# hulu/statsd-router

Hardware: AMD Instinct MI355X
Metric: M metrics/s parsed+hashed, device-resident (GiB/s and HBM roofline alongside) (higher is better)
Workload: dtype u64

## Files before the change

### statsd-router_amd/csrc/route_kernel.hpp

```cpp
#pragma once

#include <hip/hip_runtime.h>
#include <stdint.h>

#include "../../include/sr_route.h"

namespace srk {

constexpr int kBlock = 256;
constexpr int kLaneBytes = 64;
constexpr int kTile = kBlock * kLaneBytes;
constexpr int kOverlay = 16;
constexpr int kNone = 0x1FFFF;
constexpr int kSpinBudget = 1 << 14;
constexpr uint32_t kFlagAgg = 1u, kFlagIncl = 2u;
constexpr uint16_t kRoutePending = 0xFFFCu;
constexpr uint32_t kRouteDefer = 0xFFFBu;
constexpr uint64_t K = 65599ull;
constexpr int kPowLo = 64, kPowHi = 24;
constexpr int kPowInv = 4;

enum : unsigned {
    KV_UNIFORM = 0,
    KV_SEGMENTS = 1u << 22,
    KV_CHUNKS = 1u << 23,
    KV_ALIVE = 1u << 28,
    KV_PICKS = 1u << 29,
    KV_DEFER1 = 1u << 31,
    KV_DEAD1 = 1u << 27,
    KV_HIST1 = 1u << 20,
};
enum : unsigned {
    ABL_NONE = 0,
    ABL_NO_LOOKBACK = 1u << 0,
    ABL_NO_LINES = 1u << 1,
    ABL_NO_PROLOGUE = 1u << 2,
    ABL_LOAD_ONLY = 1u << 4,
    ABL_STAMPS = 1u << 5,
    ABL_NO_HASH = 1u << 8,
    ABL_FAKE_BASE = 1u << 12,
    ABL_NO_MID_BASE = 1u << 21,
};
enum : unsigned { CH_ABL_NO_U = 1u << 24, CH_ABL_NO_SUF = 1u << 25, CH_ABL_NO_EMIT = 1u << 26 };

constexpr unsigned kKvBits = KV_SEGMENTS | KV_CHUNKS | KV_ALIVE | KV_PICKS | KV_DEFER1 | KV_DEAD1 | KV_HIST1;
constexpr unsigned kAblBits = ABL_NO_LOOKBACK | ABL_NO_LINES | ABL_NO_PROLOGUE | ABL_LOAD_ONLY | ABL_STAMPS |
                              ABL_NO_HASH | ABL_FAKE_BASE | ABL_NO_MID_BASE;
constexpr unsigned kChAblBits = CH_ABL_NO_U | CH_ABL_NO_SUF | CH_ABL_NO_EMIT;
static_assert((kKvBits & kAblBits) == 0 && (kKvBits & kChAblBits) == 0 && (kAblBits & kChAblBits) == 0,
              "the three groups of variant flags are disjoint");
static_assert(__builtin_popcount(kKvBits) == 7 && __builtin_popcount(kAblBits) == 8 && __builtin_popcount(kChAblBits) == 3,
              "no two variant flags share a bit (one bit per flag listed above)");

template <unsigned ABL>
constexpr bool kCountsHist = (ABL & KV_ALIVE) != 0 || ((ABL & KV_DEAD1) != 0 && (ABL & KV_HIST1) != 0);

constexpr uint64_t ipow(uint64_t b, unsigned e) {
    uint64_t r = 1;
    while (e) {
        if (e & 1) r *= b;
        b *= b;
        e >>= 1;
    }
    return r;
}
constexpr uint64_t inv_odd(uint64_t a) {
    uint64_t x = a;
    for (int i = 0; i < 6; ++i) x *= 2 - a * x;
    return x;
}
constexpr uint64_t kK16 = ipow(K, 16), kK32 = ipow(K, 32), kK48 = ipow(K, 48), kK64 = ipow(K, 64);
constexpr uint64_t kK4096 = ipow(K, 4096);
constexpr uint64_t kK4 = ipow(K, 4);
constexpr int32_t kK2lo = (int32_t)(K * K - (1ull << 32));
static_assert(K * K == (1ull << 32) + 0x7E0F81ull, "K^2 split");
constexpr uint64_t kKinv = inv_odd(K);
static_assert(K * kKinv == 1ull, "K inverse");

struct Magic {
    uint64_t m;
    uint32_t shift;
    uint32_t kind;
};

struct PendingLine {
    uint32_t rec;
    uint32_t batch;
    uint64_t hash;
};

struct Control {
    uint32_t epoch;
    uint32_t pad1;
    uint32_t pending;
    uint32_t pad0[29];
    uint32_t done[8][32];
    uint64_t scan_xcc[32];
    uint32_t layout[8][32];
};

constexpr int kMaxBatches = 32;
constexpr int kHistKeys = 17;
constexpr int kPerClass = 8;
struct BatchDesc {
    const uint8_t *bytes;
    sr_record *recs;
    uint64_t *hashes;
    uint64_t *n_out;
    uint32_t nbytes;
    uint32_t max_records;
    uint32_t tile0;
    uint32_t ntiles;
    uint32_t sbase;
    uint32_t cls;
    uint32_t pad;
    uint64_t *probed_dead;
    uint64_t *dhash;
};

struct RouteParams {
    uint32_t nb;
    uint32_t total_blocks;
    uint32_t xcd_local;
    uint32_t nds;
    uint32_t dead;
    uint32_t pending_cap;
    uint32_t nwords_check;
    uint32_t nwords;
    uint32_t defer;
    uint32_t picks;
    uint32_t mark;
    uint32_t mark_tiles;
    Magic magic_n;
    const uint64_t *alive;
    const Magic *magic;
    const uint64_t *kpow;
    Control *ctl;
    uint64_t *status;
    uint64_t *bases;
    PendingLine *pending;
    uint64_t *tile_pd;
    uint64_t *dbg;
    uint32_t *layout_out;
    const uint64_t *cpow;
    uint64_t *tail;
    uint32_t lb_spin;
    uint32_t pad_lb;
    uint32_t prefetch;
    uint32_t pad_pf;
    uint64_t alive_w0;
    Magic magic_n1;
    uint32_t dead_k;
    uint32_t pad_dk;
    uint32_t *hist;
    uint32_t cls_tab[8][kPerClass];
    BatchDesc b[kMaxBatches];
};

// ... 246 lines not shown
}

constexpr uint32_t kMagicLds = kOverlay + 1;
__device__ __forceinline__ Magic magic_from_pad(const uint32_t *img, uint32_t e) {
    Magic mg;
    const uint32_t lo = img[(4 * e) * 17 + 16], hi = img[(4 * e + 1) * 17 + 16];
    mg.m = ((uint64_t)hi << 32) | lo;
    mg.shift = img[(4 * e + 2) * 17 + 16];
    mg.kind = img[(4 * e + 3) * 17 + 16];
    return mg;
}

constexpr uint32_t kAliveRow0 = 4 * kMagicLds;
constexpr uint32_t kAliveLds = 16;
__device__ __forceinline__ uint32_t alive_pad_dword(const uint32_t *img, uint32_t k) {
    return img[(kAliveRow0 + (k >> 5)) * 17 + 16];
}

constexpr uint32_t kMarkRow0 = kAliveRow0 + 2 * kAliveLds;
__device__ __forceinline__ void note_dead_lds(uint32_t *img, uint32_t k) {
    atomicOr(&img[(kMarkRow0 + (k >> 5)) * 17 + 16], 1u << (k & 31));
}

constexpr uint32_t kReplayCheckWords = 16;
__device__ __forceinline__ void note_dead_wg(uint64_t *pd, unsigned long long *wg, uint32_t k) {
    if (wg && k < 64 * kReplayCheckWords) {
        const unsigned long long bit = 1ull << (k & 63);
        if (!(wg[k >> 6] & bit)) atomicOr(&wg[k >> 6], bit);
        return;
    }
    note_dead(pd, k);
}

struct ProbeArgs {
    uint32_t nds, dead, picks, pad;
    Magic magic_n;
    const uint64_t *alive;
    const Magic *magic;
};

template <bool MARK = false, class P = RouteParams, int OV = kOverlay>
__device__ uint32_t probe_shard(uint64_t h, const P &p, uint64_t *mark = nullptr,
                                const uint32_t *pad_img = nullptr, unsigned long long *mark_wg = nullptr,
                                bool defer = false, uint32_t *mark_lds = nullptr) {
    const uint32_t n = p.nds;
    if (p.dead >= n) {
        if (MARK && n) note_all_dead(mark, n);
        return SR_ROUTE_ALL_DEAD;
    }
    if (p.dead == 0) return mod_magic(h, p.magic_n, n);
    const bool lds_alive = pad_img && n <= 64 * kAliveLds;
    const uint64_t alive0 = n > 64 ? 0ull
                            : lds_alive ? ((uint64_t)alive_pad_dword(pad_img, 32) << 32) | alive_pad_dword(pad_img, 0)
                                        : p.alive[0];
    auto alive_k = [&](uint32_t k) {
        if (n <= 64) return ((alive0 >> k) & 1ull) != 0;
        if (lds_alive) return ((alive_pad_dword(pad_img, k) >> (k & 31)) & 1u) != 0;
        return alive_bit(p.alive, k);
    };
    auto magic_i = [&](uint32_t i) {
        return (pad_img && n - i < kMagicLds) ? magic_from_pad(pad_img, n - i) : p.magic[i];
    };
    uint32_t o0 = 0xFFFFFFFFu, o1 = 0xFFFFFFFFu;
    uint32_t i = n;
    const int np = (defer && p.picks == 1) ? 1 : 2;
    for (int it = 0; it < np && i > 0; ++it, --i) {
        const uint32_t j = mod_magic(h, magic_i(i), i);
        const uint32_t k = (o0 >> 16) == j ? (o0 & 0xFFFFu) : j;
        if (alive_k(k)) return k;
        if (MARK) note_dead_wg(mark, mark_wg, k);
        if (mark_lds) note_dead_lds(mark_lds, k);
        if (j != i - 1) {
            const uint32_t v = (o0 >> 16) == i - 1 ? (o0 & 0xFFFFu) : i - 1;
            if (o0 == 0xFFFFFFFFu) o0 = (j << 16) | v;
            else o1 = (j << 16) | v;
        }
        h = (h * 7 + 5) / 3;
    }
    if (defer && i > 0) return kRouteDefer;
    static_assert(OV >= 2 && OV <= kOverlay, "overlay entries");
    uint32_t ov[OV];
    int nov = (o0 != 0xFFFFFFFFu) + (o1 != 0xFFFFFFFFu);
#pragma unroll
    for (int e = 0; e < OV; ++e) ov[e] = e == 0 ? o0 : (e == 1 ? o1 : 0xFFFFFFFFu);
    for (; i > 0; --i) {
        const uint32_t j = mod_magic(h, magic_i(i), i);
        uint32_t k = j;
#pragma unroll
        for (int e = 0; e < OV; ++e)
            if ((ov[e] >> 16) == j) k = ov[e] & 0xFFFFu;
        if (alive_k(k)) return k;
        if (MARK) note_dead_wg(mark, mark_wg, k);
        if (mark_lds) note_dead_lds(mark_lds, k);
        if (j != i - 1) {
            uint32_t v = i - 1;
#pragma unroll
            for (int e = 0; e < OV; ++e)
                if ((ov[e] >> 16) == i - 1) v = ov[e] & 0xFFFFu;
            if (nov == OV) return kRoutePending;
#pragma unroll
            for (int e = 0; e < OV; ++e)
                if (e == nov) ov[e] = (j << 16) | v;
            ++nov;
        }
        h = (h * 7 + 5) / 3;
    }
    return SR_ROUTE_ALL_DEAD;
}

__device__ __forceinline__ uint32_t chunk_probe(uint64_t h, const RouteParams &p, uint32_t *img) {
    const uint32_t n = p.nds;
    if (p.dead >= n) return SR_ROUTE_ALL_DEAD;
    if (p.dead == 0) return mod_magic(h, p.magic_n, n);
    const bool small = n <= 64;
    const uint64_t alive0 = small ? ((uint64_t)alive_pad_dword(img, 32) << 32) | alive_pad_dword(img, 0) : 0ull;
    const int np = p.dead >= 2 && p.picks == 1 ? 1 : 2;
    uint32_t o0 = 0xFFFFFFFFu;
    uint32_t i = n;
    for (int it = 0; it < np; ++it, --i) {
        const Magic mg = it == 0 ? p.magic_n : magic_from_pad(img, n - i);
        const uint32_t j = mod_magic(h, mg, i);
        const uint32_t k = (o0 >> 16) == j ? (o0 & 0xFFFFu) : j;
        const bool al = small ? ((alive0 >> k) & 1ull) != 0
                              : (n <= 64 * kAliveLds ? ((alive_pad_dword(img, k) >> (k & 31)) & 1u) != 0
                                                     : alive_bit(p.alive, k));
        if (al) return k;
        if (p.mark_tiles) note_dead_lds(img, k);
        if (j != i - 1) o0 = (j << 16) | (i - 1);
        h = (h * 7 + 5) / 3;
    }
    return kRouteDefer;
}

__device__ __forceinline__ uint32_t defer1_probe(uint64_t h, const RouteParams &p) {
    const uint32_t j = mod_magic(h, p.magic_n, p.nds);
    return ((p.alive_w0 >> j) & 1ull) ? j : kRouteDefer;
}

__device__ __forceinline__ uint32_t dead1_probe(uint64_t h, const RouteParams &p, uint32_t *img) {
    const uint32_t n = p.nds, d = p.dead_k;
    const uint32_t j = mod_magic(h, p.magic_n, n);
    if (j != d) return j;
    if (p.mark_tiles) note_dead_lds(img, d);
    const uint32_t j2 = mod_magic((h * 7 + 5) / 3, p.magic_n1, n - 1);
    return j2 == j ? n - 1 : j2;
}

template <unsigned ABL>
__device__ __forceinline__ void mark_tile_end(const RouteParams &p, const uint32_t *img, const BatchDesc &bd, uint32_t t,
                                              int tid);

template <unsigned ABL>
constexpr bool kOcc8 = (ABL & ~ABL_STAMPS) == (KV_UNIFORM | KV_ALIVE);

template <bool SLIM = false>
struct SmemT {
    typedef int32_t pos_t;
    static constexpr int kWaves = kBlock / 64;
    static constexpr int kTileB = kTile;
    static constexpr int kHalo = 2048;
    static constexpr int kWin = kBlock;
    static constexpr int kRows = (kHalo + kTileB) / 64;
    static constexpr int kWords = kRows * 17 + 20;
    uint32_t img[kWords];
    int32_t lend[kWin + 1];
    int32_t lcol[kWin + 1];
    uint32_t wave_cnt[kWaves];
    static constexpr int kSegWords = ((kTileB + kHalo) / 64 + kWin) / 64 + 4;
    uint32_t seg_w[kWaves][2];
    uint64_t seg_mask[kSegWords];
    uint32_t seg_first[kSegWords];
    uint64_t seg_carry[kSegWords];
    uint32_t wave_scan[kWaves][4];
    uint64_t kp_lo[kPowLo];
    uint64_t kp_hi[kPowHi];
    uint64_t kp_inv[kPowInv];
    static constexpr int kPowWords = (kPowLo + kPowHi + kPowInv) * 2;
    int32_t s_pre, c_pre;
    uint32_t hist[kHistKeys];
    uint32_t epoch, base;
    uint32_t scan_head, scan_pub, scan_total;
    __device__ __forceinline__ void put_pow(int w, uint32_t v) { ((uint32_t *)&kp_lo[0])[w] = v; }
    __device__ __forceinline__ uint64_t pow_rem(int r) const { return kp_lo[r]; }
};

template <>
struct SmemT<true> {
    typedef uint16_t pos_t;
    static constexpr int kWaves = kBlock / 64;
    static constexpr int kTileB = kTile;
    static constexpr int kHalo = 1536;
    static constexpr int kWin = kBlock;
    static constexpr int kRows = (kHalo + kTileB) / 64;
    static constexpr int kWords = kRows * 17 + 20;
    static constexpr int kPowWords = (kPowLo + kPowHi) * 2;
    static_assert(kHalo >= (int)SR_MAX_LINE_LENGTH - 1 && kHalo % 64 == 0 && kHalo >= 512, "halo holds every valid straddler");
    static_assert(kTileB < 0xFFFF, "16-bit tile positions");
    static_assert(kPowWords <= kRows, "power tables in the pad dwords");
    uint32_t img[kWords];
    uint64_t kp_rem[4];
    uint16_t lend[kWin + 1];
    uint16_t lcol[kWin + 1];
    uint32_t wave_cnt[kWaves];
    uint32_t wave_scan[kWaves][4];
    int32_t s_pre, c_pre;
    uint32_t hist[kHistKeys];
    uint32_t epoch, base;
    uint32_t scan_head, scan_pub, scan_total;
    __device__ __forceinline__ void put_pow(int w, uint32_t v) {
        img[w * 17 + 16] = v;
        if (w < 8) ((uint32_t *)&kp_rem[0])[w] = v;
    }
    __device__ __forceinline__ uint64_t pow_rem(int r) const { return kp_rem[r]; }
    __device__ __forceinline__ uint64_t pow_lo(int i) const {
        return ((uint64_t)img[(2 * i + 1) * 17 + 16] << 32) | img[(2 * i) * 17 + 16];
    }
    __device__ __forceinline__ uint64_t pow_hi(int i) const { return pow_lo(kPowLo + i); }
};
static_assert(sizeof(SmemT<true>) <= 20480, "eight workgroups per CU: 160 KiB of LDS");

template <class S>
__device__ __forceinline__ uint64_t kpow_n(const S &sm, int n) {
    return sm.kp_hi[n >> 6] * sm.kp_lo[n & 63];
}
__device__ __forceinline__ uint64_t kpow_n(const SmemT<true> &sm, int n) {
    return sm.pow_hi(n >> 6) * sm.pow_lo(n & 63);
}

__device__ __forceinline__ int img_dw(int b) { return (b >> 6) * 17 + ((b >> 2) & 15); }

template <class S>
__device__ __forceinline__ uint64_t sdbm_img(const S &sm, int a, int n, const uint64_t *slot = nullptr,
                                             uint64_t *st = nullptr) {
    const int lead = a & 3, L = lead + n;
    const int F = L >> 2, rem = L & 3;
    const int dw = a >> 2, s16 = dw & 15, cross = 16 - s16;
    const uint32_t *const p = &sm.img[(dw >> 4) * 17 + s16];
    const uint32_t first = p[0] & (0xFFFFFFFFu << (8 * lead));
    if (F == 0) return sdbm_dword_fast(0, first << (8 * (4 - rem)));
    uint64_t h = sdbm_dword_fast(0, first);
    int m = 1;
    const int F1 = F < cross ? F : cross;
    for (; m + 3 < F1; m += 4)
        h = sdbm_qword_fast(sdbm_qword_fast(h, p[m], p[m + 1]), p[m + 2], p[m + 3]);
    for (; m < F1; ++m) h = sdbm_dword_fast(h, p[m]);
    if (slot) *st = __hip_atomic_load(slot, __ATOMIC_RELAXED, __HIP_MEMORY_SCOPE_AGENT);
    for (; m + 3 < F; m += 4)
        h = sdbm_qword_fast(sdbm_qword_fast(h, p[m + 1], p[m + 2]), p[m + 3], p[m + 4]);
    for (; m < F; ++m) h = sdbm_dword_fast(h, p[m + 1]);
    if (rem) h = h * sm.pow_rem(rem) + sdbm_dword_fast(0, p[m + (m >= cross ? 1 : 0)] << (8 * (4 - rem)));
    return h;
}

__device__ __forceinline__ uint32_t lds_addr(const void *p) {
    return (uint32_t)(uintptr_t)(const __attribute__((address_space(3))) void *)p;
}
template <int O0, int O1>
__device__ __forceinline__ void ds_write2_at(uint32_t base, uint32_t a, uint32_t b) {
    asm volatile("ds_write2_b32 %0, %1, %2 offset0:%3 offset1:%4" ::"v"(base), "v"(a), "v"(b), "i"(O0), "i"(O1)
                 : "memory");
}

template <class S>
__device__ __forceinline__ void img_put16(S &sm, int b, uint4 v) {
    const int i = img_dw(b);
    sm.img[i] = v.x;
    sm.img[i + 1] = v.y;
    sm.img[i + 2] = v.z;
    sm.img[i + 3] = v.w;
}
template <class S>
__device__ __forceinline__ uint4 img_get16(const S &sm, int b) {
    const int i = img_dw(b);
    return make_uint4(sm.img[i], sm.img[i + 1], sm.img[i + 2], sm.img[i + 3]);
}

__device__ uint32_t count_tile_wave(uint32_t nbytes, __amdgpu_buffer_rsrc_t rsrc, uint32_t m, int lane) {
    constexpr uint32_t T = kTile;
    uint32_t c = 0;
    for (uint32_t off = lane * 16; off < T; off += 1024) {
        const uint4 v = load16(rsrc, m * T + off, nbytes);
        c += eq_count4(v.x, 0x0A0A0A0Au) + eq_count4(v.y, 0x0A0A0A0Au) + eq_count4(v.z, 0x0A0A0A0Au) +
             eq_count4(v.w, 0x0A0A0A0Au);
    }
    return (uint32_t)wave_sum64(c);
}

constexpr uint32_t kFlagBase = 2u;
constexpr uint32_t kFlagXcc = 3u;
constexpr uint32_t kCountMask = 0x0FFFFFFFu;

__device__ __forceinline__ uint32_t xcc_id() {
    uint32_t x;
    asm volatile("s_getreg_b32 %0, hwreg(HW_REG_XCC_ID, 0, 4)" : "=s"(x));
    return x;
}

__device__ __forceinline__ void granule_store(uint64_t *slot, uint64_t v, bool same_xcd) {
    if (same_xcd)
        __hip_atomic_store(slot, v, __ATOMIC_RELAXED, __HIP_MEMORY_SCOPE_WORKGROUP);
    else
        __hip_atomic_store(slot, v, __ATOMIC_RELAXED, __HIP_MEMORY_SCOPE_AGENT);
}

__device__ __forceinline__ bool granule_ok(uint64_t st, uint32_t ep, uint32_t flag) {
    return (uint32_t)(st >> 34) == ep && ((st >> 32) & 3u) == flag;
}

__device__ __forceinline__ uint32_t stamp_block(const RouteParams &p, const BatchDesc &bd, uint32_t t) {
    return p.xcd_local ? (bd.tile0 + t) * 8u + bd.cls : bd.tile0 + t;
}

template <unsigned ABL, class S>
__device__ void scan_batch_split(const RouteParams &p, const BatchDesc &bd, uint32_t epoch, S &sm,
                                 int wave, int lane) {
    constexpr uint32_t kRing = 4096;
    static_assert(S::kWords >= (int)kRing, "scanner ring in the LDS image");
    uint32_t *const ring = sm.img;
    if (wave == 0) {
        const uint64_t *status = p.status + bd.sbase;
        const __amdgpu_buffer_rsrc_t rsrc =
            __builtin_amdgcn_make_buffer_rsrc((void *)bd.bytes, (short)0, (int)bd.nbytes, 0x00020000);
        const uint32_t ep = epoch & 0x3FFFFFFFu;
        const uint32_t mine = (8u | xcc_id()) << 28;
        if (lane == 0)
            __hip_atomic_store(&p.ctl->scan_xcc[blockIdx.x], mk_status(epoch, kFlagXcc, xcc_id()), __ATOMIC_RELAXED,
                               __HIP_MEMORY_SCOPE_AGENT);
        uint32_t run = 0, c = 0;
        int spin = 0;
        const uint32_t last = bd.ntiles - 1u;
        auto poll = [&](uint32_t c0) -> uint64_t {
            const uint32_t tt = c0 + lane < last ? c0 + lane : last;
            return __hip_atomic_load(&status[tt], __ATOMIC_RELAXED, __HIP_MEMORY_SCOPE_AGENT);
        };
        auto step = [&](uint64_t cur, uint32_t ccur, uint64_t &nxt, uint32_t &cnxt) {
            while (c + 64 > __hip_atomic_load(&sm.scan_pub, __ATOMIC_ACQUIRE, __HIP_MEMORY_SCOPE_WORKGROUP) + kRing)
                __builtin_amdgcn_s_sleep(1);
            cnxt = c;
            nxt = poll(c);
            const int sh = (int)(c - ccur);
            uint64_t st = cur;
            if (sh) {
                const int src = (lane + sh) & 63;
                st = ((uint64_t)(uint32_t)__shfl((int)(uint32_t)(cur >> 32), src) << 32) |
                     (uint32_t)__shfl((int)(uint32_t)cur, src);
            }
            const uint32_t tt = c + lane;
            uint32_t cnt = 0, loc = 0;
            bool have = tt >= bd.ntiles;
            if (!have && lane + sh < 64 && granule_ok(st, ep, kFlagAgg)) {
                cnt = (uint32_t)st & kCountMask;
                loc = ((uint32_t)st & ~kCountMask) == mine && mine ? 0x80000000u : 0u;
                have = true;
            }
            if (spin >= kSpinBudget) {
                uint64_t missing = __ballot(!have);
                while (missing) {
                    const int L = __builtin_ctzll(missing);
                    missing &= missing - 1;
                    const uint32_t c2 = count_tile_wave(bd.nbytes, rsrc, c + (uint32_t)L, lane);
                    if (lane == L) {
                        cnt = c2;
                        have = true;
                    }
                }
            }
            const uint64_t missing = __ballot(!have);
            const int nready = missing ? __builtin_ctzll(missing) : 64;
            if (nready) {
                const uint32_t v = lane < nready ? cnt : 0u;
                const uint32_t incl = wave_incl_add32(v);
                if (lane < nready && tt < bd.ntiles) {
                    ring[tt % kRing] = (run + incl - v) | loc;
                    if (ABL & ABL_STAMPS)
                        p.dbg[(size_t)stamp_block(p, bd, tt) * 16 + 13] = __builtin_amdgcn_s_memrealtime();
                }
                run += (uint32_t)__builtin_amdgcn_readlane((int)incl, 63);
                c += (uint32_t)nready;
                if (c > bd.ntiles) c = bd.ntiles;
                spin = 0;
                if (lane == 0) {
                    if (c >= bd.ntiles) sm.scan_total = run;
                    __hip_atomic_store(&sm.scan_head, c, __ATOMIC_RELEASE, __HIP_MEMORY_SCOPE_WORKGROUP);
                }
            } else {
                ++spin;
                __builtin_amdgcn_s_sleep(1);
            }
        };
        uint64_t pa = poll(0), pb = 0;
        uint32_t ca = 0, cb = 0;
        while (c < bd.ntiles) {
            step(pa, ca, pb, cb);
            if (c >= bd.ntiles) break;
            step(pb, cb, pa, ca);
        }
    } else if (wave == 1) {
        uint64_t *const bases = p.bases + bd.sbase;
        uint32_t pub = 0;
        while (pub < bd.ntiles) {
            const uint32_t h = __hip_atomic_load(&sm.scan_head, __ATOMIC_ACQUIRE, __HIP_MEMORY_SCOPE_WORKGROUP);
            if (h == pub) {
                __builtin_amdgcn_s_sleep(1);
                continue;
// ... 249 lines not shown
        if (t > 0 && !(ABL & ABL_NO_PROLOGUE) && fm) {
            const int L = 63 - __builtin_clzll(fm);
            const int pos = (int)__builtin_amdgcn_readlane(fb + 31 - __builtin_clz(nl8 | 1u), L);
            s_abs = T0 - kHalo + pos + 1;
            const int b0 = pos + 1 - fb;
            const uint32_t keep = b0 <= 0 ? 0xFFu : (b0 >= 8 ? 0u : (0xFFu & ~((1u << b0) - 1u)));
            const uint32_t cm8 = (eq_mask4(y0, 0x3A3A3A3Au) | (eq_mask4(y1, 0x3A3A3A3Au) << 4)) & keep;
            const uint64_t cb = __ballot(cm8 != 0);
            if (cb) {
                const int Lc = __builtin_ctzll(cb);
                c_pre = (int)__builtin_amdgcn_readlane(fb + __builtin_ctz(cm8 | 0x100u), Lc) - kHalo;
            }
        } else if (t > 0 && !(ABL & ABL_NO_PROLOGUE)) {
            static_assert(kHalo <= 2048 && kHalo % 32 == 0, "32 halo bytes per lane");
            const bool in_halo = 32 * lane < kHalo;
            const uint4 a0 = img_get16(sm, 32 * lane), a1 = img_get16(sm, 32 * lane + 16);
            const uint32_t nl32 = in_halo ? eq_mask16(a0, 0x0A0A0A0Au) | (eq_mask16(a1, 0x0A0A0A0Au) << 16) : 0u;
            const uint64_t m = __ballot(nl32 != 0);
            if (m) {
                const int L = 63 - __builtin_clzll(m);
                const int pos = (int)__builtin_amdgcn_readlane(32 * lane + 31 - __builtin_clz(nl32 | 1u), L);
                s_abs = T0 - kHalo + pos + 1;
            } else {
                int64_t hi = T0 - kHalo;
                uint64_t mm = 0;
                int64_t a = 0;
                uint32_t nl16 = 0;
                while (hi > 0 && !mm) {
                    const int64_t lo = hi - 1024 > 0 ? hi - 1024 : 0;
                    a = lo + lane * 16;
                    nl16 = 0;
                    if (a < hi) nl16 = eq_mask16(load16(rsrc, (uint32_t)a, nbytes), 0x0A0A0A0Au);
                    mm = __ballot(nl16 != 0);
                    hi = lo;
                }
                if (mm) {
                    const int L = 63 - __builtin_clzll(mm);
                    s_abs = (int64_t)readlane64((uint64_t)(a + 31 - __builtin_clz(nl16 | 1u)), L) + 1;
                }
            }
            const int s_rel = (int)(s_abs - T0);
            if (s_rel < 0 && -s_rel <= (int)SR_MAX_LINE_LENGTH - 1) {
                const int b0 = kHalo + s_rel - 32 * lane;
                const uint32_t keep = !in_halo ? 0u : b0 <= 0 ? 0xFFFFFFFFu : (b0 >= 32 ? 0u : ~((1u << b0) - 1u));
                const uint32_t cm = (eq_mask16(a0, 0x3A3A3A3Au) | (eq_mask16(a1, 0x3A3A3A3Au) << 16)) & keep;
                const uint64_t cb = __ballot(cm != 0);
                if (cb) {
                    const int L = __builtin_ctzll(cb);
                    const int pos = (int)__builtin_amdgcn_readlane(32 * lane + __builtin_ctz(cm | 0x80000000u), L);
                    c_pre = pos - kHalo;
                }
            }
        }
        if (lane == 0) {
            sm.s_pre = (int32_t)(s_abs - T0);
            sm.c_pre = c_pre;
        }
    }

    auto stage = [&](int wbase, uint64_t nl, uint64_t cl, int lf, int ofc) {
        const int nc = __popcll(nl);
        if (nl && lf + nc > wbase && lf < wbase + kWin) {
            uint64_t m = nl;
            int idx = lf;
            int prevb = -1;
            while (m) {
                const int b = __builtin_ctzll(m);
                m &= m - 1;
                int c;
                if (prevb < 0 && ofc != kNone) {
                    c = ofc;
                } else {
                    const uint64_t below = b == 0 ? 0ull : (~0ull >> (64 - b));
                    const uint64_t above = ~0ull << (prevb + 1);
                    const uint64_t cm = cl & below & above;
                    c = cm ? o + __builtin_ctzll(cm) : kNone;
                }
                if (idx >= wbase && idx < wbase + kWin) {
                    sm.lend[idx - wbase + 1] = (pos_t)(o + b);
                    sm.lcol[idx - wbase + 1] = (pos_t)c;
                }
                ++idx;
                prevb = b;
            }
        }
    };
    if (tid == 0) sm.lend[0] = 0;
    uint32_t base = (ABL & ABL_FAKE_BASE) ? t * tile_count : 0u;
    bool have_base = (ABL & (ABL_NO_LOOKBACK | ABL_NO_LINES | ABL_FAKE_BASE)) != 0;
    if (tile_count > 0) {
        if (!multi_any && (int)tile_count <= kWin) {
            if (nlm) {
                const int b = __builtin_ctzll(nlm);
                const uint64_t cm = clm & (b == 0 ? 0ull : (~0ull >> (64 - b)));
                sm.lend[lane_first + 1] = (pos_t)(o + b);
                sm.lcol[lane_first + 1] = (pos_t)(open_fc != kNone ? open_fc : (cm ? o + __builtin_ctzll(cm) : kNone));
            }
        } else {
            stage(0, nlm, clm, lane_first, open_fc);
        }
    }
    for (int wbase = 0; wbase < (int)tile_count;) {
        wg_barrier();
        if (wbase == 0) stamp<ABL>(p, tid, g, 4);
        uint64_t st_early = 0;
        if (!(ABL & ABL_NO_LINES)) {
            const int s_pre = sm.s_pre;
            const int c_pre = sm.c_pre;
            const int nwin = min(kWin, (int)tile_count - wbase);
            int G = 1;
            while (G < 32 && (G * 64 + 1) * (int)tile_count <= kTileB) G <<= 1;
            auto finish = [&](int j, int s, int len, bool len_ok, bool fmt_ok, uint64_t h) {
                uint32_t route;
                if (!len_ok) route = SR_ROUTE_INVALID_LENGTH;
                else if (!fmt_ok) route = SR_ROUTE_INVALID_FORMAT;
                else if (ABL & KV_ALIVE) route = p.nds ? mod_magic(h, p.magic_n, p.nds) : SR_ROUTE_ALL_DEAD;
                else if (ABL & KV_DEFER1) route = defer1_probe(h, p);
                else if (ABL & KV_DEAD1) route = dead1_probe(h, p, sm.img);
                else if (ABL & KV_PICKS) route = chunk_probe(h, p, sm.img);
                else route = probe_shard(h, p, nullptr, sm.img, nullptr, p.defer != 0,
                                         p.mark_tiles ? sm.img : nullptr);
                const bool deferred = !(ABL & KV_ALIVE) && route == kRouteDefer;
                if (deferred) route = kRoutePending;
                sr_record r;
                r.offset = (uint32_t)(T0 + s);
                r.length = len > 0xFFFF ? (uint16_t)0xFFFF : (uint16_t)len;
                r.route = (uint16_t)route;
                if (!have_base) {
                    stamp<ABL>(p, tid, g, 3);
                    base = granule_ok(st_early, epoch & 0x3FFFFFFFu, kFlagBase)
                               ? (uint32_t)st_early
                               : wait_base(base_slot, epoch, rsrc, (uint32_t)T0);
                    stamp<ABL>(p, tid, g, 7);
                    have_base = true;
                }
                const uint32_t rec = base + (uint32_t)j;
                if (rec < bd.max_records) {
                    if constexpr (kCountsHist<ABL>)
                        if (p.hist) atomicAdd(&sm.hist[route < p.nds ? route : p.nds], 1u);
                    if (deferred) bd.dhash[rec] = h;
                    if (!(ABL & (KV_ALIVE | KV_DEFER1 | KV_DEAD1)) && route == kRoutePending && !deferred) {
                        const uint32_t slot = atomicAdd(&p.ctl->pending, 1u);
                        if (slot < p.pending_cap) p.pending[slot] = PendingLine{rec, bi, h};
                    }
                    bd.recs[rec] = r;
                    if (bd.hashes) bd.hashes[rec] = h;
                }
            };
            auto line_at = [&](int j, int e, int c, int s, bool act, int gi, int Gl, int Gw) {
                const int len = e - s + 1;
                const bool len_ok = len >= (int)SR_MIN_LINE_LENGTH && len <= (int)SR_MAX_LINE_LENGTH;
                const bool fmt_ok = c != kNone && c < e;
                uint64_t h = 0;
                if (act && len_ok && fmt_ok && !(ABL & ABL_NO_HASH)) {
                    const int n = c - s, nseg = (n + 63) >> 6;
                    for (int k = gi; k < nseg; k += Gl) {
                        const int a = s + 64 * k, nn = min(64, n - 64 * k);
                        const bool mid = !(ABL & ABL_NO_MID_BASE) && !have_base && k == gi;
                        uint64_t hs = sdbm_img(sm, a + kHalo, nn, mid ? base_slot : nullptr, &st_early);
                        if (k + 1 < nseg) hs *= kpow_n(sm, c - a - nn);
                        h += hs;
                    }
                }
                for (int d = Gw >> 1; d >= 1; d >>= 1) {
                    const uint64_t v = shfl_xor64(h, d);
                    if (d < Gl) h += v;
                }
                if (act && gi == 0) finish(j, s, len, len_ok, fmt_ok, h);
            };
            auto line = [&](int jj, bool act, int gi, int Gl, int Gw) {
                const int j = wbase + jj;
                const int e = act ? sm.lend[jj + 1] : 0;
                int c = act ? sm.lcol[jj + 1] : kNone;
                if (j == 0 && c_pre != kNone) c = c_pre;
                const int s = (j == 0) ? s_pre : (act ? sm.lend[jj] + 1 : 0);
                line_at(j, e, c, s, act, gi, Gl, Gw);
            };
            bool segs = false;
            bool gain2 = false;
            uint32_t TL = 0;
            const bool last_win = wbase + kWin >= (int)tile_count;
            if constexpr ((ABL & KV_SEGMENTS) != 0) if (last_win) {
                uint32_t want = 0, nsg = 0;
                if (tid < nwin) {
                    const int jj = tid, j = wbase + jj;
                    const int e = sm.lend[jj + 1];
                    int c = sm.lcol[jj + 1];
                    if (j == 0 && c_pre != kNone) c = c_pre;
                    const int s = (j == 0) ? s_pre : sm.lend[jj] + 1;
                    const int len = e - s + 1;
                    if (len >= (int)SR_MIN_LINE_LENGTH && len <= (int)SR_MAX_LINE_LENGTH && c != kNone && c < e)
                        nsg = (uint32_t)(c - s + 63) >> 6;
                    want = max(1u, nsg);
                }
                const uint32_t incl = wave_incl_add32(want);
                const uint32_t wmx = wave_incl_max32(nsg);
                if (lane == 63) {
                    sm.seg_w[wave][0] = incl;
                    sm.seg_w[wave][1] = wmx;
                }
                if (tid < 2 * S::kSegWords) reinterpret_cast<uint32_t *>(sm.seg_mask)[tid] = 0u;
                wg_barrier();
                uint32_t pre = 0, mx = 0, tot = 0;
#pragma unroll
                for (int w = 0; w < kWaves; ++w) {
                    const uint32_t v = sm.seg_w[w][0];
                    tot += v;
                    pre += w < wave ? v : 0u;
                    mx = max(mx, sm.seg_w[w][1]);
                }
                TL = __builtin_amdgcn_readfirstlane(tot);
                const uint32_t mxs = (uint32_t)__builtin_amdgcn_readfirstlane(mx);
                const int cost_u = ((nwin * G + kBlock - 1) / kBlock) * (int)((mxs + (uint32_t)G - 1) / (uint32_t)G);
                const int cost_s = ((int)TL + kBlock - 1) / kBlock;
                segs = cost_s < cost_u;
                gain2 = cost_s + 2 <= cost_u;
                if (segs) {
                    if (tid < nwin) {
                        const uint32_t wn = want;
                        const uint32_t st = pre + incl - want;
                        atomicOr(&sm.seg_mask[st >> 6], 1ull << (st & 63));
                        const uint32_t m = (st + 63) & ~63u;
                        if (m < st + wn) sm.seg_first[m >> 6] = (st << 16) | (uint32_t)tid;
                    }
                    wg_barrier();
                }
            }
            if (wbase == 0) stamp<ABL>(p, tid, g, 14);
            if ((ABL & KV_SEGMENTS) && last_win && tid == 0) {
                __hip_atomic_fetch_add(&p.ctl->layout[g & 7u][0], 1u, __ATOMIC_RELAXED, __HIP_MEMORY_SCOPE_AGENT);
                if (gain2)
                    __hip_atomic_fetch_add(&p.ctl->layout[g & 7u][1], 1u, __ATOMIC_RELAXED, __HIP_MEMORY_SCOPE_AGENT);
            }
            if (!segs) {
                for (int r0 = 0; r0 < nwin * G; r0 += kBlock) {
                    const uint32_t x = (uint32_t)(r0 + tid);
                    const int jj = (int)(x >> __builtin_ctz((unsigned)G));
                    line(jj, jj < nwin, (int)(x & (uint32_t)(G - 1)), G, G);
                }
            } else if constexpr ((ABL & KV_SEGMENTS) != 0) {
                for (int r0 = 0; r0 < (int)TL; r0 += kBlock) {
                    const uint32_t x = (uint32_t)(r0 + tid);
                    const uint32_t k = x >> 6;
                    const bool act = x < TL;
                    const bool live = r0 + wave * 64 < (int)TL;
                    uint64_t below = 0, part = 0;
                    int sg = 0, glast = -1, j = 0, s = 0, len = 0;
                    bool len_ok = false, fmt_ok = false;
                    if (live) {
                        const uint64_t mask = readlane64(act ? sm.seg_mask[k] : 0ull, 0);
                        const uint32_t fst = (uint32_t)__builtin_amdgcn_readfirstlane(act ? sm.seg_first[k] : 0u);
                        below = mask & (~0ull >> (63 - lane));
                        const int hb = below ? 63 - __clzll(below) : -1;
                        const int jj = (int)(fst & 0xFFFFu) + __popcll(below) - (int)(mask & 1ull);
                        sg = below ? lane - hb : (int)(x - (fst >> 16));
                        j = wbase + jj;
                        const int e = act ? sm.lend[jj + 1] : 0;
                        int c = act ? sm.lcol[jj + 1] : kNone;
                        if (j == 0 && c_pre != kNone) c = c_pre;
                        s = (j == 0) ? s_pre : (act ? sm.lend[jj] + 1 : 0);
                        len = e - s + 1;
                        len_ok = len >= (int)SR_MIN_LINE_LENGTH && len <= (int)SR_MAX_LINE_LENGTH;
                        fmt_ok = c != kNone && c < e;
                        const int n = c - s;
                        const int nseg = (act && len_ok && fmt_ok) ? (n + 63) >> 6 : 0;
                        glast = act ? max(nseg, 1) - 1 : -1;
                        uint64_t hs = 0;
                        if (sg < nseg) {
                            const int a = s + 64 * sg, nn = min(64, n - 64 * sg);
                            const bool mid = !have_base && sg == nseg - 1;
                            hs = sdbm_img(sm, a + kHalo, nn, mid ? base_slot : nullptr, &st_early);
                            if (sg + 1 < nseg) hs *= kpow_n(sm, c - a - nn);
                        }
                        const uint64_t Sx = wave_scan64(hs, 0ull, [](uint64_t l, uint64_t r) { return l + r; });
                        const int src = hb > 0 ? hb - 1 : 0;
                        const uint64_t Sb = ((uint64_t)(uint32_t)__shfl((int)(Sx >> 32), src, 64) << 32) |
                                            (uint32_t)__shfl((int)(uint32_t)Sx, src, 64);
                        part = hb > 0 ? Sx - Sb : Sx;
                        if (lane == 63 && act && sg < glast) sm.seg_carry[k] = part;
                    }
                    wg_barrier();
                    if (sg == glast) {
                        const uint64_t h = below ? part : part + sm.seg_carry[k - 1];
                        finish(j, s, len, len_ok, fmt_ok, h);
                    }
                }
            }
        }

        wg_barrier();
        if (wbase == 0) stamp<ABL>(p, tid, g, 5);
        if (wbase + kWin >= (int)tile_count) break;
        if (tid == 0) sm.lend[0] = sm.lend[kWin];
        wg_barrier();
        wbase += kWin;
        {
            const uint32_t *const row = &sm.img[(kHalo / 64 + tid) * 17];
            uint32_t m[4];
#pragma unroll
            for (int k = 0; k < 4; ++k) m[k] = nl_colon_mask16(make_uint4(row[4 * k], row[4 * k + 1], row[4 * k + 2], row[4 * k + 3]));
            const uint64_t nl = ((uint64_t)__builtin_amdgcn_perm(m[3], m[2], 0x05040100u) << 32) |
                                __builtin_amdgcn_perm(m[1], m[0], 0x05040100u);
            const uint64_t cl = ((uint64_t)__builtin_amdgcn_perm(m[3], m[2], 0x07060302u) << 32) |
                                __builtin_amdgcn_perm(m[1], m[0], 0x07060302u);
            const uint32_t cin = wave_incl_add32((uint32_t)__popcll(nl));
            const uint32_t kin = wave_incl_min32(((8191u - cin) << 17) | lane_cand(nl, cl));
            int lf, ofc;
            lane_state(cin, kin, lf, ofc);
            stage(wbase, nl, cl, lf, ofc);
        }
    }
    }
    stamp<ABL>(p, tid, g, 6);
}

template <int BLOCK, unsigned ABL>
__global__ __launch_bounds__(kBlock, (KernelTraits<ABL>::kMinWavesPerSimd))
__attribute__((amdgpu_waves_per_eu((KernelTraits<ABL>::kMinWavesPerSimd), (KernelTraits<ABL>::kMaxWavesPerSimd)))) void route_kernel(RouteParams p) {
    static_assert(BLOCK == kBlock, "one workgroup size");
    using S = SmemT<kOcc8<ABL>>;
    __shared__ S sm;
    const int tid = threadIdx.x;
    const int lane = tid & 63;
    const int wave = tid >> 6;
    uint4 hdr;
    const uint32_t bi = launch_header_batch(hdr);
    if (blockIdx.x < hdr.x) {
        __builtin_amdgcn_s_setprio(3);
        if (uint64_t *pd = p.b[blockIdx.x].probed_dead)
            for (uint32_t w = tid; w < p.nwords; w += kBlock) pd[w] = 0ull;
        const uint32_t ep0 = __hip_atomic_load(&p.ctl->epoch, __ATOMIC_RELAXED, __HIP_MEMORY_SCOPE_AGENT);
        if (tid == 0) {
            sm.scan_head = 0;
            sm.scan_pub = 0;
            sm.scan_total = 0;
        }
        wg_barrier();
        scan_batch_split<ABL>(p, p.b[blockIdx.x], ep0, sm, wave, lane);
        if (tid == 64) arrive(p, blockIdx.x, ep0);
        return;
    }
    const uint32_t g = blockIdx.x - hdr.x;
    stamp<ABL>(p, tid, g, 8);
    if ((ABL & ABL_STAMPS) && tid == 0) {
        uint32_t hw;
        asm volatile("s_getreg_b32 %0, hwreg(HW_REG_HW_ID)" : "=s"(hw));
        p.dbg[(size_t)g * 16 + 10] = hw;
        p.dbg[(size_t)g * 16 + 11] = xcc_id();
    }
    if (bi >= kMaxBatches) {
        if (tid == 0) arrive(p, blockIdx.x, __hip_atomic_load(&p.ctl->epoch, __ATOMIC_RELAXED, __HIP_MEMORY_SCOPE_AGENT));
        return;
    }
    const uint32_t t = (hdr.z ? (g >> 3) : g) - p.b[bi].tile0;
    TileIn in;
    tile_issue<ABL>(p, bi, t, in, tid);
    const uint32_t kp = tid < S::kPowWords ? ((const uint32_t *)p.kpow)[tid] : 0u;
    in.sx = __hip_atomic_load(&p.ctl->scan_xcc[bi], __ATOMIC_RELAXED, __HIP_MEMORY_SCOPE_AGENT);
    const uint32_t ep0 = __hip_atomic_load(&p.ctl->epoch, __ATOMIC_RELAXED, __HIP_MEMORY_SCOPE_AGENT);
    if (kEarlyArrive<ABL> && tid == 0) arrive_count_after(p, blockIdx.x, ep0);
    if (tid < S::kPowWords) sm.put_pow(tid, kp);
    if (!(ABL & (KV_ALIVE | KV_DEFER1 | KV_DEAD1)) && p.dead && p.dead < p.nds && tid < 4 * (int)kMagicLds) {
        const uint32_t e = (uint32_t)tid >> 2;
        if (e < p.nds) sm.img[(uint32_t)tid * 17 + 16] = ((const uint32_t *)&p.magic[p.nds - e])[tid & 3];
    }
    if (!(ABL & (KV_ALIVE | KV_DEFER1 | KV_DEAD1)) && p.dead && p.dead < p.nds && p.nds <= 64 * kAliveLds && tid >= (int)kAliveRow0 &&
        (uint32_t)tid < kAliveRow0 + 2 * ((p.nds + 63) / 64))
        sm.img[(uint32_t)tid * 17 + 16] = ((const uint32_t *)p.alive)[tid - kAliveRow0];
    if (!(ABL & (KV_ALIVE | KV_DEFER1)) && p.mark_tiles && tid >= (int)kMarkRow0 && (uint32_t)tid < kMarkRow0 + 2 * p.nwords)
        sm.img[(uint32_t)tid * 17 + 16] = 0u;
    if (tid < 20) sm.img[S::kRows * 17 + tid] = 0u;
    if (kCountsHist<ABL> && p.hist && tid < kHistKeys) sm.hist[tid] = 0u;
    uint64_t nlm, clm;
    uint32_t c_in;
    tile_load<ABL>(p, sm, in, ep0, g, nlm, clm, c_in);
    tile_lines<ABL>(p, sm, in, ep0, g, nlm, clm, c_in);
    mark_tile_end<ABL>(p, sm.img, p.b[bi], t, tid);
    if (kCountsHist<ABL> && p.hist) {
        wg_barrier();
        const BatchDesc &bd = p.b[bi];
        if ((uint32_t)tid <= p.nds)
            p.hist[(size_t)(p.nds + 1) * bd.sbase + (size_t)tid * bd.ntiles + t] = sm.hist[tid];
    }
    if (tid == 0) {
        if (kEarlyArrive<ABL>) arrive_last(p, blockIdx.x, ep0);
        else arrive(p, blockIdx.x, ep0);
    }
    stamp<ABL>(p, tid, g, 9);
}

template <unsigned ABL>
__device__ __forceinline__ void mark_tile_end(const RouteParams &p, const uint32_t *img, const BatchDesc &bd, uint32_t t,
                                              int tid) {
    if ((ABL & (KV_ALIVE | KV_DEFER1)) || !p.mark_tiles || !bd.probed_dead) return;
    wg_barrier();
    if ((uint32_t)tid < p.nwords) {
        const uint32_t lo = img[(kMarkRow0 + 2 * (uint32_t)tid) * 17 + 16];
        const uint32_t hi = img[(kMarkRow0 + 2 * (uint32_t)tid + 1) * 17 + 16];
        p.tile_pd[(size_t)(bd.sbase + t) * p.nwords + tid] = ((uint64_t)hi << 32) | lo;
    }
}

constexpr uint32_t kProbePads = (kAliveRow0 + 2 * kAliveLds) * 17;
template <class P>
__device__ __forceinline__ bool probe_pad_value(const P &p, uint32_t tid, uint32_t &v) {
    if (tid < 4 * kMagicLds && (tid >> 2) < p.nds) {
        v = ((const uint32_t *)&p.magic[p.nds - (tid >> 2)])[tid & 3];
        return true;
    }
    if (p.nds <= 64 * kAliveLds && tid >= kAliveRow0 && tid < kAliveRow0 + 2 * ((p.nds + 63) / 64)) {
        v = ((const uint32_t *)p.alive)[tid - kAliveRow0];
        return true;
    }
    return false;
}
__device__ __forceinline__ void load_probe_pads(const RouteParams &p, uint32_t *pads, uint32_t tid) {
    uint32_t v;
    if (probe_pad_value(p, tid, v)) pads[tid * 17 + 16] = v;
}

constexpr uint32_t kDeferChunk = 256;
constexpr uint32_t kDeferOrBlocks = 16;
template <int OV>
__global__ __launch_bounds__(256) void probe_defer_kernel(RouteParams p) {
    __shared__ uint32_t pads[kProbePads];
    __shared__ uint32_t list[4][kDeferChunk];
    __shared__ unsigned long long wg[kReplayCheckWords];
    const uint32_t bi = blockIdx.y;
    if (bi >= p.nb) return;
    const BatchDesc &bd = p.b[bi];
    const uint32_t tid = threadIdx.x, lane = tid & 63u, w = tid >> 6;
    uint64_t *const mark = p.mark ? bd.probed_dead : nullptr;
    const uint32_t n = (uint32_t)min(*bd.n_out, (uint64_t)bd.max_records);
    uint32_t pv = 0;
    const bool has_pv = probe_pad_value(p, tid, pv);
    const uint32_t nor = min(gridDim.x, kDeferOrBlocks);
    uint64_t v0 = 0;
    if (mark && p.mark_tiles && blockIdx.x < nor)
        for (uint32_t t = blockIdx.x * 256u + tid; t < bd.ntiles; t += nor * 256u)
            v0 |= p.tile_pd[(size_t)(bd.sbase + t) * p.nwords];
    if (blockIdx.x >= nor && blockIdx.x * 4u * kDeferChunk >= n) return;
    const uint32_t x0 = (blockIdx.x * 4u + w) * kDeferChunk + lane;
    uint16_t r0[kDeferChunk / 64];
#pragma unroll
    for (uint32_t it = 0; it < kDeferChunk / 64; ++it) {
        const uint32_t x = x0 + 64u * it;
        r0[it] = (p.defer && x < n) ? bd.recs[x].route : (uint16_t)0;
    }
    if (has_pv) pads[tid * 17 + 16] = pv;
    if (tid < kReplayCheckWords) wg[tid] = 0ull;
    __syncthreads();
    if (mark && p.mark_tiles && blockIdx.x < nor) {
        if (v0) atomicOr(&wg[0], (unsigned long long)v0);
        for (uint32_t q = 1; q < p.nwords; ++q) {
            uint64_t v = 0;
            for (uint32_t t = blockIdx.x * 256u + tid; t < bd.ntiles; t += nor * 256u)
                v |= p.tile_pd[(size_t)(bd.sbase + t) * p.nwords + q];
            if (v) atomicOr(&wg[q], (unsigned long long)v);
        }
    }
    const uint64_t below = (1ull << lane) - 1ull;
    bool first = true;
    for (uint32_t c = blockIdx.x * 4u + w; p.defer && c * kDeferChunk < n; c += gridDim.x * 4u) {
        const uint32_t xc = c * kDeferChunk + lane;
        uint16_t r[kDeferChunk / 64];
#pragma unroll
        for (uint32_t it = 0; it < kDeferChunk / 64; ++it) {
            const uint32_t x = xc + 64u * it;
            r[it] = x < n ? (first ? r0[it] : bd.recs[x].route) : (uint16_t)0;
        }
        first = false;
        uint32_t cnt = 0;
#pragma unroll
        for (uint32_t it = 0; it < kDeferChunk / 64; ++it) {
            const uint64_t m = __ballot(r[it] == kRoutePending);
            if (r[it] == kRoutePending) list[w][cnt + __popcll(m & below)] = xc + 64u * it;
            cnt += __popcll(m);
        }
        __builtin_amdgcn_wave_barrier();
        uint32_t xs[kDeferChunk / 64];
        uint64_t hs[kDeferChunk / 64];
#pragma unroll
        for (uint32_t it = 0; it < kDeferChunk / 64; ++it) {
            const uint32_t i = lane + 64u * it;
            xs[it] = i < cnt ? list[w][i] : 0u;
            hs[it] = i < cnt ? bd.dhash[xs[it]] : 0ull;
        }
#pragma unroll
        for (uint32_t it = 0; it < kDeferChunk / 64; ++it) {
            if (lane + 64u * it >= cnt) break;
            const uint32_t x = xs[it];
            const uint64_t h = hs[it];
            const uint32_t route = mark ? probe_shard<true, RouteParams, OV>(h, p, mark, pads, wg)
                                        : probe_shard<false, RouteParams, OV>(h, p, nullptr, pads);
            if (route == kRoutePending) {
                const uint32_t slot = atomicAdd(&p.ctl->pending, 1u);
                if (slot < p.pending_cap) p.pending[slot] = PendingLine{x, bi, h};
            }
            bd.recs[x].route = (uint16_t)route;
        }
        __builtin_amdgcn_wave_barrier();
    }
    if (mark) {
        __syncthreads();
        if (tid < p.nwords && wg[tid])
            __hip_atomic_fetch_or(mark + tid, (uint64_t)wg[tid], __ATOMIC_RELAXED, __HIP_MEMORY_SCOPE_AGENT);
    }
}

__global__ __launch_bounds__(64) void probe_wide_kernel(RouteParams p) {
    extern __shared__ uint16_t ds_index[];
    const uint32_t n = p.nds;
    for (uint32_t i = threadIdx.x; i < n; i += blockDim.x) ds_index[i] = (uint16_t)i;
    __syncthreads();
    const uint32_t np = min(__hip_atomic_load(&p.ctl->pending, __ATOMIC_RELAXED, __HIP_MEMORY_SCOPE_AGENT),
                            p.pending_cap);
    if (threadIdx.x != 0) return;
    for (uint32_t x = blockIdx.x; x < np; x += gridDim.x) {
        const PendingLine pl = p.pending[x];
        uint64_t h = pl.hash;
        uint32_t route = SR_ROUTE_ALL_DEAD, steps = 0;
        for (uint32_t i = n; i > 0; --i) {
            const uint32_t j = mod_magic(h, p.magic[i], i);
            const uint32_t k = ds_index[j];
            ++steps;
            if (alive_bit(p.alive, k)) { route = k; break; }
            if (p.b[pl.batch].probed_dead) note_dead(p.b[pl.batch].probed_dead, k);
            if (j != i - 1) {
                ds_index[j] = ds_index[i - 1];
                ds_index[i - 1] = (uint16_t)k;
            }
            h = (h * 7 + 5) / 3;
        }
        p.b[pl.batch].recs[pl.rec].route = (uint16_t)route;
        h = pl.hash;
        for (uint32_t i = n; i > 0 && steps > 0; --i, --steps) {
            const uint32_t j = mod_magic(h, p.magic[i], i);
            ds_index[j] = (uint16_t)j;
            ds_index[i - 1] = (uint16_t)(i - 1);
// ... 76 lines not shown
```

Before: 58490.

## Compute SDBM key hashes with int8 MFMA matrix ops on occupancy-8 path

Reformulates the polynomial SDBM hash of each 64-byte key segment as an int8 matrix product. The powers of K are split into signed byte digits and stored in LDS pad dwords, and mfma_i32_16x16x64_i8 produces partial sums that are recombined into a 64-bit hash. Alignment to 16-byte boundaries is undone afterwards by multiplying by a power of the inverse of K. The aim is to move the serial 64-bit multiply-add chain onto the matrix cores. It also pins the epoch and tile index in scalar registers to relieve VGPR pressure, at the cost of wave-wide ballot loops and masking work for short keys.

```diff
diff --git a/statsd-router_amd/csrc/route_kernel.hpp b/statsd-router_amd/csrc/route_kernel.hpp
--- a/statsd-router_amd/csrc/route_kernel.hpp
+++ b/statsd-router_amd/csrc/route_kernel.hpp
@@ -4,6 +4,10 @@
 #include <stdint.h>
 
 #include "../../include/sr_route.h"
+
+#ifndef SR_SDBM_MFMA
+#define SR_SDBM_MFMA 1
+#endif
 
 namespace srk {
 
@@ -556,6 +560,8 @@
 
 template <unsigned ABL>
 constexpr bool kOcc8 = (ABL & ~ABL_STAMPS) == (KV_UNIFORM | KV_ALIVE);
+template <unsigned ABL>
+constexpr bool kMx = SR_SDBM_MFMA != 0 && kOcc8<ABL>;
 
 template <bool SLIM = false>
 struct SmemT {
@@ -654,6 +660,111 @@
     for (; m < F; ++m) h = sdbm_dword_fast(h, p[m + 1]);
     if (rem) h = h * sm.pow_rem(rem) + sdbm_dword_fast(0, p[m + (m >= cross ? 1 : 0)] << (8 * (4 - rem)));
     return h;
+}
+
+typedef int v4i32 __attribute__((ext_vector_type(4)));
+constexpr int kMxPowRow = 0;
+constexpr int kMxInvRow = 2 * kPowHi;
+constexpr int kMxWRow = kMxInvRow + 32;
+constexpr int kMxRows = kMxWRow + 8 * 5 * 4;
+static_assert(kMxRows <= SmemT<true>::kRows && kMxRows <= kBlock, "the matrix-core tables in the pad dwords, one per thread");
+
+constexpr int mx_digit(uint64_t v, int l) {
+    int d = 0;
+    for (int i = 0; i <= l; ++i) {
+        d = (int)(v & 0xFFu);
+        if (d >= 128) d -= 256;
+        v = (v - (uint64_t)(int64_t)d) >> 8;
+    }
+    return d;
+}
+struct MxTab {
+    uint32_t w[kMxRows];
+};
+constexpr MxTab make_mx_tab() {
+    MxTab t{};
+    for (int i = 0; i < kPowHi; ++i) {
+        const uint64_t v = ipow(K, 64u * (unsigned)i);
+        t.w[kMxPowRow + 2 * i] = (uint32_t)v;
+        t.w[kMxPowRow + 2 * i + 1] = (uint32_t)(v >> 32);
+    }
+    for (int z = 0; z < 16; ++z) {
+        const uint64_t v = ipow(kKinv, (unsigned)z);
+        t.w[kMxInvRow + 2 * z] = (uint32_t)v;
+        t.w[kMxInvRow + 2 * z + 1] = (uint32_t)(v >> 32);
+    }
+    for (int m = 0; m < 4; ++m)
+        for (int half = 0; half < 2; ++half)
+            for (int r = 0; r < 4; ++r)
+                for (int j = 0; j < 16; ++j) {
+                    const int d = mx_digit(ipow(K, (unsigned)(63 - 16 * m - j)), 4 * half + r);
+                    t.w[kMxWRow + ((2 * m + half) * 5 + r) * 4 + (j >> 2)] |= (uint32_t)(d & 0xFF) << (8 * (j & 3));
+                }
+    return t;
+}
+__device__ const MxTab kMxTab = make_mx_tab();
+
+__device__ __forceinline__ uint64_t mx_combine(v4i32 a, v4i32 b) {
+    const int32_t p01 = a[0] + (int32_t)((uint32_t)a[1] << 8), p23 = a[2] + (int32_t)((uint32_t)a[3] << 8);
+    const uint32_t p45 = (uint32_t)b[0] + ((uint32_t)b[1] << 8), p67 = (uint32_t)b[2] + ((uint32_t)b[3] << 8);
+    const uint64_t lo = (uint64_t)((int64_t)p01 + (int64_t)((uint64_t)(int64_t)p23 << 16));
+    return lo + ((uint64_t)(p45 + (p67 << 16)) << 32);
+}
+
+__device__ __forceinline__ uint32_t mx_bytemask(uint32_t nib) { return ((nib * 0x00204081u) & 0x01010101u) * 0xFFu; }
+
+template <class S>
+__device__ __forceinline__ uint64_t sdbm_mx(const S &sm, bool valid, int s_img, int c_img, int gi, int Gl,
+                                            const uint64_t *slot, uint64_t *st) {
+    const int lane = threadIdx.x & 63;
+    const int cls = (lane >> 4) == ((lane & 15) >> 2) ? (lane & 3) : 4;
+    const uint32_t *const wa = &sm.img[(kMxWRow + 4 * cls) * 17 + 16];
+    const int E = (c_img + 15) & ~15;
+    const int w0 = E - 64 * (gi + 1);
+    int f = valid ? s_img - w0 : 64;
+    int e = c_img - w0;
+    const uint32_t *row = &sm.img[(w0 >> 6) * 17 + ((w0 >> 2) & 15)];
+    const int q3 = (E >> 4) & 3;
+    uint64_t h = 0;
+    bool first = true;
+    while (__ballot(f < 64) != 0ull) {
+        const bool on = f < 64;
+        const uint32_t *const rp = on ? row : &sm.img[0];
+        const uint64_t bits = on ? (~0ull >> ((64 - min(e, 64)) & 63)) & (~0ull << (max(f, 0) & 63)) : 0ull;
+        v4i32 acc0 = {0, 0, 0, 0}, acc1 = {0, 0, 0, 0};
+#pragma unroll
+        for (int m = 0; m < 4; ++m) {
+            const uint32_t p16 = (uint32_t)(bits >> (16 * m)) & 0xFFFFu;
+            if (m == 2 && first && slot) *st = __hip_atomic_load(slot, __ATOMIC_RELAXED, __HIP_MEMORY_SCOPE_AGENT);
+            if (__ballot(p16 != 0u) == 0ull) continue;
+            const uint32_t *const pp = rp + 4 * m + ((q3 + m) >> 2);
+            v4i32 b = {(int)pp[0], (int)pp[1], (int)pp[2], (int)pp[3]};
+            if (__ballot(p16 != 0xFFFFu) != 0ull) {
+#pragma unroll
+                for (int d = 0; d < 4; ++d) b[d] &= (int)mx_bytemask((p16 >> (4 * d)) & 15u);
+            }
+            const uint32_t *const a0 = wa + (2 * m) * 20 * 17, *const a1 = wa + (2 * m + 1) * 20 * 17;
+            const v4i32 A0 = {(int)a0[0], (int)a0[17], (int)a0[34], (int)a0[51]};
+            acc0 = __builtin_amdgcn_mfma_i32_16x16x64_i8(A0, b, acc0, 0, 0, 0);
+            const v4i32 A1 = {(int)a1[0], (int)a1[17], (int)a1[34], (int)a1[51]};
+            acc1 = __builtin_amdgcn_mfma_i32_16x16x64_i8(A1, b, acc1, 0, 0, 0);
+        }
+        uint64_t v = mx_combine(acc0, acc1);
+        if (e > 64) {
+            const int k = (e - 1) >> 6;
+            v *= ((uint64_t)sm.img[(kMxPowRow + 2 * k + 1) * 17 + 16] << 32) | sm.img[(kMxPowRow + 2 * k) * 17 + 16];
+        }
+        h += v;
+        f += 64 * Gl;
+        e += 64 * Gl;
+        row -= 17 * Gl;
+        first = false;
+    }
+    return h;
+}
+template <class S>
+__device__ __forceinline__ uint64_t mx_kinv(const S &sm, int z) {
+    return ((uint64_t)sm.img[(kMxInvRow + 2 * z + 1) * 17 + 16] << 32) | sm.img[(kMxInvRow + 2 * z) * 17 + 16];
 }
 
 __device__ __forceinline__ uint32_t lds_addr(const void *p) {
@@ -1209,7 +1320,11 @@
                 const bool len_ok = len >= (int)SR_MIN_LINE_LENGTH && len <= (int)SR_MAX_LINE_LENGTH;
                 const bool fmt_ok = c != kNone && c < e;
                 uint64_t h = 0;
-                if (act && len_ok && fmt_ok && !(ABL & ABL_NO_HASH)) {
+                if constexpr (kMx<ABL>) {
+                    const bool mid = !(ABL & ABL_NO_MID_BASE) && !have_base;
+                    h = sdbm_mx(sm, act && len_ok && fmt_ok, s + kHalo, c + kHalo, gi, Gl, mid ? base_slot : nullptr,
+                                &st_early);
+                } else if (act && len_ok && fmt_ok && !(ABL & ABL_NO_HASH)) {
                     const int n = c - s, nseg = (n + 63) >> 6;
                     for (int k = gi; k < nseg; k += Gl) {
                         const int a = s + 64 * k, nn = min(64, n - 64 * k);
@@ -1223,7 +1338,11 @@
                     const uint64_t v = shfl_xor64(h, d);
                     if (d < Gl) h += v;
                 }
-                if (act && gi == 0) finish(j, s, len, len_ok, fmt_ok, h);
+                if (act && gi == 0) {
+                    if constexpr (kMx<ABL>)
+                        if (len_ok && fmt_ok) h *= mx_kinv(sm, -(c + kHalo) & 15);
+                    finish(j, s, len, len_ok, fmt_ok, h);
+                }
             };
             auto line = [&](int jj, bool act, int gi, int Gl, int Gw) {
                 const int j = wbase + jj;
@@ -1412,11 +1531,16 @@
     const uint32_t t = (hdr.z ? (g >> 3) : g) - p.b[bi].tile0;
     TileIn in;
     tile_issue<ABL>(p, bi, t, in, tid);
-    const uint32_t kp = tid < S::kPowWords ? ((const uint32_t *)p.kpow)[tid] : 0u;
+    const uint32_t kp = kMx<ABL> ? (tid < kMxRows ? kMxTab.w[tid] : 0u)
+                                 : (tid < S::kPowWords ? ((const uint32_t *)p.kpow)[tid] : 0u);
     in.sx = __hip_atomic_load(&p.ctl->scan_xcc[bi], __ATOMIC_RELAXED, __HIP_MEMORY_SCOPE_AGENT);
     const uint32_t ep0 = __hip_atomic_load(&p.ctl->epoch, __ATOMIC_RELAXED, __HIP_MEMORY_SCOPE_AGENT);
     if (kEarlyArrive<ABL> && tid == 0) arrive_count_after(p, blockIdx.x, ep0);
-    if (tid < S::kPowWords) sm.put_pow(tid, kp);
+    if constexpr (kMx<ABL>) {
+        if (tid < kMxRows) sm.img[tid * 17 + 16] = kp;
+    } else {
+        if (tid < S::kPowWords) sm.put_pow(tid, kp);
+    }
     if (!(ABL & (KV_ALIVE | KV_DEFER1 | KV_DEAD1)) && p.dead && p.dead < p.nds && tid < 4 * (int)kMagicLds) {
         const uint32_t e = (uint32_t)tid >> 2;
         if (e < p.nds) sm.img[(uint32_t)tid * 17 + 16] = ((const uint32_t *)&p.magic[p.nds - e])[tid & 3];
@@ -1431,17 +1555,24 @@
     uint64_t nlm, clm;
     uint32_t c_in;
     tile_load<ABL>(p, sm, in, ep0, g, nlm, clm, c_in);
-    tile_lines<ABL>(p, sm, in, ep0, g, nlm, clm, c_in);
-    mark_tile_end<ABL>(p, sm.img, p.b[bi], t, tid);
+    uint32_t ep1 = ep0, te = t;
+    if constexpr (kMx<ABL>) ep1 = (uint32_t)__builtin_amdgcn_readfirstlane((int)ep0);
+    tile_lines<ABL>(p, sm, in, ep1, g, nlm, clm, c_in);
+    if constexpr (kMx<ABL>) {
+        uint32_t g2 = g;
+        asm volatile("" : "+s"(g2));
+        te = (hdr.z ? (g2 >> 3) : g2) - p.b[bi].tile0;
+    }
+    mark_tile_end<ABL>(p, sm.img, p.b[bi], te, tid);
     if (kCountsHist<ABL> && p.hist) {
         wg_barrier();
         const BatchDesc &bd = p.b[bi];
         if ((uint32_t)tid <= p.nds)
-            p.hist[(size_t)(p.nds + 1) * bd.sbase + (size_t)tid * bd.ntiles + t] = sm.hist[tid];
+            p.hist[(size_t)(p.nds + 1) * bd.sbase + (size_t)tid * bd.ntiles + te] = sm.hist[tid];
     }
     if (tid == 0) {
-        if (kEarlyArrive<ABL>) arrive_last(p, blockIdx.x, ep0);
-        else arrive(p, blockIdx.x, ep0);
+        if (kEarlyArrive<ABL>) arrive_last(p, blockIdx.x, ep1);
+        else arrive(p, blockIdx.x, ep1);
     }
     stamp<ABL>(p, tid, g, 9);
 }
```

After: 61980 (median of 6 runs). 6.0% higher.
